# PH8411/image-matching

Measured on AMD Instinct MI355X. Metric: image-pairs/sec (640x480, 1024 kpts, 30 Sinkhorn iters), higher is better.
Workload: dtype f32

## Files before the change

### image-matching_amd/csrc/conv1ab_wino24p.hip

```cpp
#include "imx_kernels.h"
#include "wino24_h2.h"
#include <cstdint>
#include <cstdio>
#include <cstdlib>
#include <type_traits>

namespace imx {

typedef float f32x4 __attribute__((ext_vector_type(4)));
typedef float f32x2 __attribute__((ext_vector_type(2)));
typedef _Float16 f16x8 __attribute__((ext_vector_type(8)));
typedef _Float16 f16x2 __attribute__((ext_vector_type(2)));
typedef unsigned u32x4v __attribute__((ext_vector_type(4)));

namespace {
constexpr int IMG_N = IMG_H * IMG_W;

__global__ __launch_bounds__(512) void conv1ab_wino24p(ConvArgs p, int tiles_x, int tiles_y, int ntiles) {
  extern __shared__ __attribute__((aligned(16))) unsigned char smem_1p[];
  float* raw = reinterpret_cast<float*>(smem_1p + NG * VGRP * 2);
  float* img = raw + NG * RAWSZ;
  float* wmax = img + NG * IMG_N;
  unsigned* amax_tab = reinterpret_cast<unsigned*>(wmax + 8);
  const unsigned lds0 = (unsigned)(uintptr_t)(__attribute__((address_space(3))) unsigned char*)smem_1p;
// ... 271 lines not shown
    f32x4 y[2][4];
    {
      auto cols = [&](const f32x4 (&a0)[3], const f32x4 (&a1)[3], const f32x4 (&b0)[3], const f32x4 (&b1)[3]) __attribute__((always_inline)) {
        const f32x4 s0[6] = {a0[0], a0[1], a0[2], b0[0], b0[1], b0[2]}, s1[6] = {a1[0], a1[1], a1[2], b1[0], b1[1], b1[2]};
        w24_out_cols(s0, s1, k8, y);
      };
      if (ph == 0) { cols(sK0, sK1, gs0, gs1); asm volatile("" ::: "memory"); }
      else { cols(gs0, gs1, sK0, sK1); asm volatile("; order 1" ::: "memory"); }
    }
    {
      const float inv = p.u_scale_inv / sv;
      const f32x4 inv4 = {inv, inv, inv, inv};
      const f32x4 zero4 = {0.f, 0.f, 0.f, 0.f};
      const int wr = (lq & 15) >> 2, wc = lq & 3;
      const int bu = __builtin_amdgcn_readfirstlane(bcur), lv = __builtin_amdgcn_readfirstlane(lcur);
      const __amdgpu_buffer_rsrc_t ors = __builtin_amdgcn_make_buffer_rsrc((void*)(p.out + (size_t)bu * Ho * Wo * Cout), 0, lv ? Ho * Wo * Cout * 4 : 0, 0x00020000);
      const int choff = outb ? (cb * 2 + (lq >> 5)) * (Ho * Wo * 32) + ((lq >> 4) & 1) * 16 : (cb * 16 + 4 * (lq >> 4)) * 4;
      typedef unsigned u32x4 __attribute__((__vector_size__(4 * sizeof(unsigned))));
      const int oy = (y0 >> 1) + wr;
#pragma unroll
      for (int hh = 0; hh < 2; ++hh) {
        const f32x4 mx4 = __builtin_elementwise_max(__builtin_elementwise_max(y[0][2 * hh], y[0][2 * hh + 1]), __builtin_elementwise_max(y[1][2 * hh], y[1][2 * hh + 1]));
        const f32x4 v = __builtin_elementwise_max(__builtin_elementwise_fma(mx4, inv4, bs4), zero4);
        const int ox = (x0 >> 1) + 2 * wc + hh;
        const unsigned off = (oy < Ho && ox < Wo) ? (unsigned)((oy * Wo + ox) * opx + choff) : 0x7ffffff0u;
        __builtin_amdgcn_raw_buffer_store_b128(__builtin_bit_cast(u32x4, v), ors, (int)off, 0, 0);
        amax_run = max(amax_run, __builtin_bit_cast(unsigned, fmaxf(fmaxf(v[0], v[1]), fmaxf(v[2], v[3]))));
      }
      if (p.amax_out) {
        unsigned mb = amax_run;
        mb = max(mb, (unsigned)__builtin_amdgcn_update_dpp(0, (int)mb, 0xb1, 0xf, 0xf, true));
        mb = max(mb, (unsigned)__builtin_amdgcn_update_dpp(0, (int)mb, 0x4e, 0xf, 0xf, true));
        mb = max(mb, (unsigned)__builtin_amdgcn_update_dpp(0, (int)mb, 0x141, 0xf, 0xf, true));
        mb = max(mb, (unsigned)__builtin_amdgcn_update_dpp(0, (int)mb, 0x140, 0xf, 0xf, true));
        const unsigned m01 = max((unsigned)__builtin_amdgcn_readlane((int)mb, 0), (unsigned)__builtin_amdgcn_readlane((int)mb, 16));
        const unsigned m23 = max((unsigned)__builtin_amdgcn_readlane((int)mb, 32), (unsigned)__builtin_amdgcn_readlane((int)mb, 48));
        const unsigned mw = max(m01, m23);
        if (lv && mw && lq == 0) atomicMax(amax_tab + (bu & (AMAX_SLOTS - 1)), mw);
        amax_run = 0;
      }
// ... 38 lines not shown
```

### image-matching_amd/csrc/conv3x3_wino24p.hip

```cpp
#include "imx_kernels.h"
#include "wino24_h2.h"
#include <cstdint>
#include <cstdio>
#include <cstdlib>
#include <type_traits>

namespace imx {

typedef float f32x4 __attribute__((ext_vector_type(4)));
typedef float f32x2 __attribute__((ext_vector_type(2)));
typedef _Float16 f16x8 __attribute__((ext_vector_type(8)));
typedef _Float16 f16x2 __attribute__((ext_vector_type(2)));
typedef unsigned u32x4 __attribute__((ext_vector_type(4)));

namespace {
#ifdef P_TRACE
__device__ long long p_trace_buf[16 * 16];
#define P_STAMP(i_) { const long long t_ = __builtin_amdgcn_s_memtime(); tr[i_] += t_ - tlast; tlast = t_; }
#else
#define P_STAMP(i_)
#endif

struct Tile { int b, y0, x0, live; };
__device__ __forceinline__ float v_scale_inv(unsigned amax_bits) {
  unsigned e = (amax_bits >> 23) & 0xffu;
  e = e < 60u ? 60u : e > 200u ? 200u : e;
  return __builtin_bit_cast(float, (e - 8u) << 23);
}

template <bool POOL, bool RELU, bool FASTW, bool INZ>
__global__ __launch_bounds__(512) void conv3x3_wino24p(ConvArgs p, int tiles_x, int tiles_y, int ntiles, int nitems) {
  extern __shared__ __attribute__((aligned(16))) unsigned char smem_p[];
  float* raw = reinterpret_cast<float*>(smem_p + NG * VGRP * 2);
  unsigned* amax_tab = reinterpret_cast<unsigned*>(raw + NG * NSUB * RAWC);
  const unsigned lds0 = (unsigned)(uintptr_t)(__attribute__((address_space(3))) unsigned char*)smem_p;

  const int tid = threadIdx.x, lane = tid & 63;
  const int wave_s = __builtin_amdgcn_readfirstlane(tid >> 6);
  const int cb = wave_s & 3, ph = wave_s >> 2;
  const int tq = wave_s & 3, tg = wave_s >> 2;
  const int H = p.H, W = p.W, Cin = p.Cin, Cout = p.Cout;
  const int nchunk = Cin / CKH, ncob = Cout / NT;
  const int grid = (int)gridDim.x;
  const int vb = (grid & 7) == 0 ? ((int)blockIdx.x & 7) * (grid >> 3) + ((int)blockIdx.x >> 3) : (int)blockIdx.x;
  if (vb >= nitems) return;
// ... 17 lines not shown
    unsigned a = lds0 + (unsigned)(ph * (VGRP * 2) + ph * NLP * 1024 + lane * 16);
    unsigned b = lds0 + (unsigned)((1 - ph) * (VGRP * 2) + ph * NLP * 1024 + lane * 16);
    asm volatile("" : "+v"(a), "+v"(b));
    vrdK = (const _Float16*)((__attribute__((address_space(3))) unsigned char*)(uintptr_t)a);
    vrdS = (const _Float16*)((__attribute__((address_space(3))) unsigned char*)(uintptr_t)b);
  }

  auto loader_slot = [&](int t, int k, int& py, int& px_, int& half) __attribute__((always_inline)) {
    const int e = (k == 1 && t + 256 < RH * RW * 2) ? t + 256 : t;
    const int px = p.in_blocked ? e >> 1 : e % (RH * RW);
    half = p.in_blocked ? e & 1 : e / (RH * RW);
    py = px / RW - 1;
    px_ = px % RW - 1;
    return px * RSC + half * 4;
  };
  constexpr bool inz = INZ;
  auto halo_slot = [&](int t, int j, int& py, int& px_, int& piece) __attribute__((always_inline)) -> bool {
    const int hh = t + 256 * j, hp = hh >> 3;
    piece = hh & 7;
    py = hp < 18 ? 0 : hp < 36 ? RH - 1 : hp < 44 ? hp - 35 : hp - 43;
    px_ = hp < 18 ? hp : hp < 36 ? hp - 18 : hp < 44 ? 0 : RW - 1;
    return hh < 52 * 8;
  };
  int ldst[2], ldmain = 0;
  if constexpr (inz) {
    const int t = tid & 255, n = t & 15, kq = (t >> 4) & 3, x = t >> 6;
    ldmain = tg * NSUB * RAWC + (kq >> 1) * RAWC + ((1 + 2 * (n >> 2)) * RW + 1 + 4 * (n & 3) + x) * RSC + (kq & 1) * 4;
#pragma unroll
    for (int j = 0; j < 2; ++j) {
      int py, px, piece;
      halo_slot(t, j, py, px, piece);
      ldst[j] = tg * NSUB * RAWC + ((piece >> 2) * 2 + ((piece & 3) >> 1)) * RAWC + (py * RW + px) * RSC + (piece & 1) * 4;
    }
  } else {
#pragma unroll
    for (int k = 0; k < 2; ++k) { int a, b, c; ldst[k] = tg * NSUB * RAWC + loader_slot(tid & 255, k, a, b, c); }
  }
  const int cob = __builtin_amdgcn_readfirstlane(vb % ncob);
  const int dt = NG * (grid / ncob), dtx = __builtin_amdgcn_readfirstlane(dt % tiles_x), dty = __builtin_amdgcn_readfirstlane((dt / tiles_x) % tiles_y),
            dtb = __builtin_amdgcn_readfirstlane(dt / (tiles_x * tiles_y));
  Tile cur, nxt;
  {
// ... 19 lines not shown
  const int nblk_in = Cin / 16;
  const int zimg = tiles_x * tiles_y * nblk_in * 8192;
  const bool inb = p.in_blocked != 0;
  const int pxb = inb ? 8 * 4 : Cin * 4;
  const int sub_step = inb ? H * W * 8 * 4 : 8 * 4;
  auto loader_tile = [&](const Tile& t) __attribute__((always_inline)) {
    const int t8 = (wave_s & 3) * 64 + lane_now();
    int lpy[2], lpx[2], lhalf[2];
#pragma unroll
    for (int k = 0; k < 2; ++k) loader_slot(t8, k, lpy[k], lpx[k], lhalf[k]);
    const bool lv = t.live != 0;
    const int b = __builtin_amdgcn_readfirstlane(lv ? t.b : 0);
    lsv = v_scale(amax_c[b & (AMAX_SLOTS - 1)]);
    if constexpr (inz) {
      lrs = __builtin_amdgcn_make_buffer_rsrc((void*)(p.in + (size_t)b * (zimg >> 2)), 0, lv ? zimg : 0, 0x00020000);
      const int n = t8 & 15, x = t8 >> 6;
      gmain = (unsigned)((t.y0 * tiles_x + t.x0) * nblk_in * 8192 + t8 * 16);
      const bool xin = t.x0 * OW + 4 * (n & 3) + x < W;
      const int gy0 = t.y0 * OH + 2 * (n >> 2);
      mmask = ((xin && gy0 < H) ? 5u : 0u) | ((xin && gy0 + 1 < H) ? 10u : 0u);
#pragma unroll
      for (int j = 0; j < 2; ++j) {
        int py, px, piece;
        const bool used = halo_slot(t8, j, py, px, piece);
        const int gy = t.y0 * OH - 1 + py, gx = t.x0 * OW - 1 + px;
        const bool in = (int)used & (int)lv & (int)((unsigned)gy < (unsigned)H) & (int)((unsigned)gx < (unsigned)W);
        goff[j] = in ? (unsigned)((((gy >> 3) * tiles_x + (gx >> 4)) * nblk_in + (piece >> 2)) * 8192 + ((gy & 1) * 4 + (gx & 3)) * 1024 + (piece & 3) * 256 +
                                  (((gy & 7) >> 1) * 4 + ((gx & 15) >> 2)) * 16)
                     : OOB;
      }
      return;
    }
    lrs = __builtin_amdgcn_make_buffer_rsrc((void*)(p.in + (size_t)b * H * W * Cin), 0, lv ? img_bytes : 0, 0x00020000);
#pragma unroll
    for (int k = 0; k < 2; ++k) {
      const int gy = t.y0 * OH + lpy[k], gx = t.x0 * OW + lpx[k];
      const bool in = (int)lv & (int)((unsigned)gy < (unsigned)H) & (int)((unsigned)gx < (unsigned)W);
      goff[k] = in ? (unsigned)((gy * W + gx) * pxb + lhalf[k] * 16) : OOB;
    }
  };
  f32x4 rr[NSUB][2];
  float rr_sv = 1.f;
  unsigned rr_mask = 0xfu;
  auto issue_load = [&]() __attribute__((always_inline)) {
// ... 17 lines not shown
  };
  auto advance_loader = [&]() __attribute__((always_inline)) {
    if (__builtin_expect(++lchunk == nchunk, 0)) {
      lchunk = 0;
      nxt = step_tile(cur);
      if (item_c + grid >= nitems) nxt.live = 0;
      loader_tile(nxt);
      asm volatile("" ::: "memory");
    }
  };
  auto store_raw = [&]() __attribute__((always_inline)) {
    const f32x4 s4 = {rr_sv, rr_sv, rr_sv, rr_sv};
    if constexpr (inz) {
#pragma unroll
      for (int k = 0; k < 4; ++k) {
        const float mk = (rr_mask >> k) & 1u ? 1.f : 0.f;
        const f32x4 v = rr[k][0] * s4 * (f32x4){mk, mk, mk, mk};
        float* d = raw + ldmain + (k & 1) * (RW * RSC) + (k >> 1) * (2 * RAWC);
        *reinterpret_cast<f32x2*>(d) = (f32x2){v[0], v[1]};
        *reinterpret_cast<f32x2*>(d + 2) = (f32x2){v[2], v[3]};
      }
      const int t8 = (wave_s & 3) * 64 + lane_now();
#pragma unroll
      for (int j = 0; j < 2; ++j)
        if (t8 + 256 * j < 52 * 8) {
          const f32x4 v = rr[j][1] * s4;
          float* d = raw + ldst[j];
          *reinterpret_cast<f32x2*>(d) = (f32x2){v[0], v[1]};
          *reinterpret_cast<f32x2*>(d + 2) = (f32x2){v[2], v[3]};
        }
      return;
    }
#pragma unroll
// ... 182 lines not shown
      };
      if (ph == 0) { cols(sK0, sK1, gs0, gs1); asm volatile("" ::: "memory"); }
      else { cols(gs0, gs1, sK0, sK1); asm volatile("; order 1" ::: "memory"); }
    }
    P_STAMP(7)
    {
      const int lwr = (lq & 15) >> 2, lwc = lq & 3;
      const int chl = outb ? (cb * 2 + (lq >> 5)) * (Ho_k * Wo_k * 8 * 4) + ((lq >> 4) & 1) * 16 : (cb * 16 + 4 * (lq >> 4)) * 4;
      const f32x4 inv4 = {inv, inv, inv, inv};
      const f32x4 zero4 = {0.f, 0.f, 0.f, 0.f};
      const int Ho = Ho_k, Wo = Wo_k;
      typedef unsigned su32x4 __attribute__((__vector_size__(4 * sizeof(unsigned))));
      const int ibase = __builtin_amdgcn_readfirstlane(((POOL ? tl.y0 >> 1 : tl.y0) * Wo + (POOL ? tl.x0 >> 1 : tl.x0)) * opx +
                                                       (outb ? cob * (NT / 8) * (Ho * Wo * 8 * 4) : cob * NT * 4));
      const int fbase = fastw ? ibase : 0;
      const bool outz = !POOL && p.out_blocked == 2;
      const int zbase = outz ? __builtin_amdgcn_readfirstlane((((tl.y0 / OH) * tiles_x + tl.x0 / OW) * (Cout / 16) + cob * 4 + cb) * 8192) : 0;
      const size_t zimg_out = (size_t)tiles_x * tiles_y * (Cout / 16) * 2048;
      const __amdgpu_buffer_rsrc_t ors =
          outz ? __builtin_amdgcn_make_buffer_rsrc((void*)(p.out + (size_t)tl.b * zimg_out + (zbase >> 2)), 0, tl.live ? 8192 : 0, 0x00020000)
               : __builtin_amdgcn_make_buffer_rsrc((void*)(p.out + (size_t)tl.b * Ho * Wo * Cout + (fbase >> 2)), 0, tl.live ? Ho * Wo * Cout * 4 - fbase : 0, 0x00020000);
      auto note = [&](const f32x4& v) __attribute__((always_inline)) {
        const float mm = RELU ? fmaxf(fmaxf(v[0], v[1]), fmaxf(v[2], v[3])) : fmaxf(fmaxf(fabsf(v[0]), fabsf(v[1])), fmaxf(fabsf(v[2]), fabsf(v[3])));
        amax_run = max(amax_run, __builtin_bit_cast(unsigned, mm));
      };
      if constexpr (POOL) {
        const int oy = (tl.y0 >> 1) + lwr;
#pragma unroll
        for (int hh = 0; hh < 2; ++hh) {
          const f32x4 mx4 = __builtin_elementwise_max(__builtin_elementwise_max(y[0][2 * hh], y[0][2 * hh + 1]), __builtin_elementwise_max(y[1][2 * hh], y[1][2 * hh + 1]));
          f32x4 v = __builtin_elementwise_fma(mx4, inv4, bs4);
          if (RELU) v = __builtin_elementwise_max(v, zero4);
          note(v);
          const int ox = (tl.x0 >> 1) + 2 * lwc + hh;
          const int so_ = (lwr * Wo + 2 * lwc + hh) * opx + chl;
          const unsigned off = fastw ? (unsigned)so_ : (oy < Ho && ox < Wo) ? (unsigned)(so_ + ibase) : OOB;
          __builtin_amdgcn_raw_buffer_store_b128(__builtin_bit_cast(su32x4, v), ors, (int)off, 0, 0);
        }
      } else {
#pragma unroll
        for (int r = 0; r < 2; ++r)
#pragma unroll
          for (int x = 0; x < 4; ++x) {
            f32x4 v = __builtin_elementwise_fma(y[r][x], inv4, bs4);
            if (RELU) v = __builtin_elementwise_max(v, zero4);
            note(v);
            const int oy = tl.y0 + 2 * lwr + r, ox = tl.x0 + 4 * lwc + x;
            const int so_ = ((2 * lwr + r) * Wo + 4 * lwc + x) * opx + chl;
            const unsigned off = outz ? (unsigned)((r * 4 + x) * 1024 + lq * 16) : fastw ? (unsigned)so_ : (oy < Ho && ox < Wo) ? (unsigned)(so_ + ibase) : OOB;
            __builtin_amdgcn_raw_buffer_store_b128(__builtin_bit_cast(su32x4, v), ors, (int)off, 0, 0);
          }
      }
      P_STAMP(13)
      if (p.amax_out) {
        unsigned mb = amax_run;
        mb = max(mb, (unsigned)__builtin_amdgcn_update_dpp(0, (int)mb, 0xb1, 0xf, 0xf, true));
        mb = max(mb, (unsigned)__builtin_amdgcn_update_dpp(0, (int)mb, 0x4e, 0xf, 0xf, true));
        mb = max(mb, (unsigned)__builtin_amdgcn_update_dpp(0, (int)mb, 0x141, 0xf, 0xf, true));
        mb = max(mb, (unsigned)__builtin_amdgcn_update_dpp(0, (int)mb, 0x140, 0xf, 0xf, true));
        const unsigned m01 = max((unsigned)__builtin_amdgcn_readlane((int)mb, 0), (unsigned)__builtin_amdgcn_readlane((int)mb, 16));
        const unsigned m23 = max((unsigned)__builtin_amdgcn_readlane((int)mb, 32), (unsigned)__builtin_amdgcn_readlane((int)mb, 48));
        const unsigned mw = max(m01, m23);
        if (tl.live && mw && lq == 0) atomicMax(amax_tab + (tl.b & (AMAX_SLOTS - 1)), mw);
        amax_run = 0;
// ... 8 lines not shown
    __syncthreads();
    for (int i = tid; i < AMAX_SLOTS; i += 512)
      if (amax_tab[i]) atomicMax(p.amax_out + i, amax_tab[i]);
  }
#ifdef P_TRACE
#ifdef P_TRACE_WAVES
  if (lane == 0 && blockIdx.x == 0)
    for (int i = 0; i < 16; ++i) p_trace_buf[wave_s * 16 + i] = tr[i];
#else
  if (tid == 0 && (blockIdx.x & 15) == 0 && (blockIdx.x >> 4) < 16)
    for (int i = 0; i < 16; ++i) p_trace_buf[(blockIdx.x >> 4) * 16 + i] = tr[i];
#endif
#endif
}

template <bool POOL, bool RELU, bool FASTW, bool INZ>
hipError_t launch_p2(const ConvArgs& a, hipStream_t s) {
  const int tiles_x = (a.W + OW - 1) / OW, tiles_y = (a.H + OH - 1) / OH;
  const int ntiles = tiles_x * tiles_y * a.B;
  const int nitems = ((ntiles + NG - 1) / NG) * (a.Cout / NT);
  const size_t lds = (size_t)NG * VGRP * 2 + (size_t)NG * NSUB * RAWC * sizeof(float) + AMAX_SLOTS * sizeof(unsigned);
  const int ncu = device_cu_count();
  if (!ncu) return hipErrorUnknown;
  auto k = conv3x3_wino24p<POOL, RELU, FASTW, INZ>;
  static unsigned long long attr = 0;
  raise_lds_limit(reinterpret_cast<const void*>(k), (int)lds, attr);
  const int ncob = a.Cout / NT;
  const dim3 grid((unsigned)(nitems <= ncu ? nitems : ncu - ncu % ncob));
  if (grid.x == 0) return hipErrorInvalidValue;
  last_form = "conv3x3_wino24p:f16x2";
  hipLaunchKernelGGL(k, grid, dim3(512), lds, s, a, tiles_x, tiles_y, ntiles, nitems);
  return hipGetLastError();
}
template <bool POOL, bool RELU, bool FASTW>
hipError_t launch_p(const ConvArgs& a, hipStream_t s) {
  return a.in_blocked == 2 ? launch_p2<POOL, RELU, FASTW, true>(a, s) : launch_p2<POOL, RELU, FASTW, false>(a, s);
}
}

#ifdef P_TRACE
void conv_p_trace_read(long long* out) { (void)hipMemcpyFromSymbol(out, HIP_SYMBOL(p_trace_buf), sizeof(long long) * 16 * 16); }
#endif

bool conv3x3_wino24p_supported(const ConvArgs& a) {
  if (!conv3x3_wino24h_supported(a)) return false;
  const size_t padded = (size_t)((a.H + OH - 1) / OH * OH) * ((a.W + OW - 1) / OW * OW) * 4;
  return padded * a.Cin < (size_t)OOB && padded * a.Cout < (size_t)OOB;
}

bool conv3x3_wino24p_preferred(const ConvArgs& a) {
  if (!conv3x3_wino24p_supported(a)) return false;
// ... 19 lines not shown
```

### image-matching_amd/csrc/imx_api.cpp

```cpp
#include "imx_host.h"

#include <dlfcn.h>

#include <atomic>
#include <memory>

namespace imx {
thread_local const char* last_form = nullptr;
}

namespace {
bool ends_with(const std::string& s, const std::string& suf) {
  return s.size() >= suf.size() && s.compare(s.size() - suf.size(), suf.size(), suf) == 0;
}
}

extern "C" {

#ifndef IMX_BUILD_ID
#define IMX_BUILD_ID "dev"
#endif
const char* imx_version(void) { return "imx 0.4 gfx950 hip-7.2 fp32 build " IMX_BUILD_ID; }

int imx_create(int device_id, const imx_config_t* cfg, imx_handle_t* out) {
// ... 409 lines not shown
    if (shape_out) for (size_t i = 0; i < it->second.shape.size() && i < 4; ++i) shape_out[i] = it->second.shape[i];
    if (!host_out) return 0;
    if (capacity < n) return fail(h, "imx_debug_fetch: capacity %lld < %lld elements", (long long)capacity, (long long)n);
    HIP_OK(h, hipSetDevice(h->device));
    HIP_OK(h, hipDeviceSynchronize());
    if (h->nms_lazy.pending && name && std::string(name) == "nms") {
      auto& z = h->nms_lazy;
      HIP_OK(h, launch_nms(z.smap, z.nms, z.B, z.H, z.W, z.radius, nullptr, z.scratch));
      HIP_OK(h, hipDeviceSynchronize());
      z.pending = false;
    }
    if (!it->second.blocked) {
      HIP_OK(h, hipMemcpy(host_out, it->second.p, (size_t)n * 4, hipMemcpyDeviceToHost));
      return 0;
    }
    std::vector<float> raw((size_t)n);
    HIP_OK(h, hipMemcpy(raw.data(), it->second.p, (size_t)n * 4, hipMemcpyDeviceToHost));
    const int64_t Bn = it->second.shape[0], Hn = it->second.shape[1], Wn = it->second.shape[2], Cn = it->second.shape[3];
    for (int64_t bb = 0; bb < Bn; ++bb)
      for (int64_t ck = 0; ck < Cn / 8; ++ck)
        for (int64_t yx = 0; yx < Hn * Wn; ++yx)
          for (int64_t c = 0; c < 8; ++c)
            host_out[(bb * Hn * Wn + yx) * Cn + ck * 8 + c] = raw[((bb * (Cn / 8) + ck) * Hn * Wn + yx) * 8 + c];
    return 0;
  });
}

int imx_set_timing(imx_handle_t h, int enable) {
  return guarded(h, "imx_set_timing", [&]() -> int {
    if (!h) return -1;
    h->timing = enable != 0;
    return 0;
  });
}

int imx_timing_reset(imx_handle_t h) {
  return guarded(h, "imx_timing_reset", [&]() -> int {
    if (!h) return -1;
// ... 62 lines not shown
```

### image-matching_amd/csrc/imx_host.h

```cpp
#pragma once
#include "../../include/imx.h"
#include "imx_kernels.h"
#include "gnn_tail_pack.h"

#include <hip/hip_runtime.h>

#include <algorithm>
#include <cstdarg>
#include <cstdio>
#include <exception>
#include <map>
#include <new>
#include <string>
#include <vector>

namespace imx::host {

constexpr int HEADS = 4;

struct HostTensor {
  std::vector<float> data;
  std::vector<int64_t> shape;
};
struct DevBuf {
// ... 19 lines not shown
  float* b = nullptr;
  int K = 0, N = 0, Npad = 0;
};
struct GnnLayer {
  GemmW qkv, merge, mlp1, mlp2;
  float* tail_stream = nullptr;
  void* tail_stream_h2 = nullptr;
  GnnTailH2Consts h2c{};
  float bmax_1 = 0.f, bmax_2 = 0.f;
  float qkv_spread = 1.f;
};
struct Tap {
  const void* p;
  std::vector<int64_t> shape;
  bool blocked = false;
};
struct TimedEvent {
  std::string name;
  const char* form;
  hipEvent_t e0, e1;
};
struct TimingRow {
  std::string name, form;
  int64_t launches;
  double ms;
};

inline std::string g_create_error;

}
// ... 211 lines not shown
```

### image-matching_amd/csrc/imx_superpoint.cpp

```cpp
#include "imx_host.h"

namespace imx::host {

namespace {

struct SpLayer { const char* name; int level; bool pool, first, last, swz; };
constexpr int kSpN = 8;
constexpr SpLayer kSpLayers[kSpN] = {{"conv1ab_pool", 0, true, true, false, false}, {"conv2a", 1, false, false, false, true},
                                  {"conv2b_pool", 1, true, false, false, false}, {"conv3a", 2, false, false, false, true},
                                  {"conv3b_pool", 2, true, false, false, false}, {"conv4a", 3, false, false, false, true},
                                  {"conv4b", 3, false, false, false, false},     {"convPaDa", 3, false, false, true, false}};
constexpr int kSlice = 256;

struct SpWork {
  int B, H, W, split;
  const float *img0, *img1;
  float* act[kSpN];
  unsigned* amax;
};
enum class ConvForm : unsigned char { Direct, Wino, WinoH, WinoP, C1, C1H, C1P };
constexpr hipError_t (*kConvLaunch[])(const ConvArgs&, hipStream_t) = {launch_conv3x3, launch_conv3x3_wino24, launch_conv3x3_wino24h, launch_conv3x3_wino24p,
                                                                       launch_conv1ab_wino24, launch_conv1ab_wino24h, launch_conv1ab_wino24p};
static_assert(sizeof(kConvLaunch) / sizeof(*kConvLaunch) == (size_t)ConvForm::C1P + 1, "one launcher per ConvForm, in the enum's order");
struct SpStep { ConvForm form; unsigned char in_blocked, out_blocked; };
struct SpPlan {
  bool blocked;
  bool chain;
  int nslice;
  int heads_cout;
  SpStep steps[2][kSpN];
};

ConvArgs conv_args(imx_handle_t h, const SpWork& w, const SpPlan& P, int li, int sl) {
  const SpLayer& T = kSpLayers[li];
  const ConvW& cw = h->conv[li];
  const int hh = w.H >> T.level, ww = w.W >> T.level, cout = T.last ? P.heads_cout : cw.cout;
  const int b0 = P.chain ? sl * kSlice : 0, nb = P.chain ? std::min(kSlice, w.B - b0) : w.B;
  const size_t ztile = (size_t)((hh + 7) / 8) * ((ww + 15) / 16) * 2048;
  const size_t in_img = li && kSpLayers[li - 1].swz ? ztile * (cw.cin / 16) : (size_t)hh * ww * (T.first ? 1 : cw.cin);
  const size_t out_img = T.swz ? ztile * (cout / 16) : (size_t)(T.pool ? hh / 2 : hh) * (T.pool ? ww / 2 : ww) * cout;
  ConvArgs a{};
  if (P.chain) {
    unsigned* am = w.amax + (size_t)sl * kSpN * 256;
    a.amax_out = T.last ? nullptr : am + (size_t)li * 256;
    a.amax_in = li > 0 ? am + (size_t)(li - 1) * 256 : nullptr;
    a.wuh = cw.wuh; a.u_scale_inv = cw.su_inv;
    a.c1a_l1 = h->c1a_l1; a.c1a_bmax = h->c1a_bmax;
  }
  a.in = (li ? w.act[li - 1] : w.img0) + (size_t)b0 * in_img;
  if (T.first) {
    if (b0 >= w.split) { a.in = w.img1 + (size_t)(b0 - w.split) * in_img; a.split = nb; }
    else { a.in2 = w.img1; a.split = w.split - b0; }
  }
  a.w = cw.w; a.wu24 = cw.wu24; a.bias = cw.b; a.w1 = h->w1; a.b1 = h->b1; a.out = w.act[li] + (size_t)b0 * out_img;
  a.B = nb; a.H = hh; a.W = ww; a.Cin = cw.cin; a.Cout = cout; a.relu = 1; a.pool = T.pool; a.first = T.first;
// ... 19 lines not shown
    const ConvArgs a = conv_args(h, w, P, kSpN - 1, 0);
    if (!conv3x3_wino24_supported(a) || (P.chain && !conv3x3_wino24h_supported(a))) P.heads_cout = h->conv[kSpN - 1].cout;
  }
  if (P.chain) P.nslice = (w.B + kSlice - 1) / kSlice;
  const bool pairs = P.chain && o.conv_f16 == 1;
  for (int r = P.nslice > 1 ? 0 : 1; r < 2; ++r) {
    SpStep* st = P.steps[r];
    for (int li = 0; li < kSpN; ++li) {
      st[li] = SpStep{};
      const ConvArgs a = conv_args(h, w, P, li, r ? P.nslice - 1 : 0);
      if (li ? !wino[li] : o.conv_direct) st[li].form = ConvForm::Direct;
      else if (li) st[li].form = !P.chain ? ConvForm::Wino : pairs && conv3x3_wino24p_preferred(a) ? ConvForm::WinoP : ConvForm::WinoH;
      else st[li].form = !(P.chain && conv1ab_wino24h_supported(a)) ? ConvForm::C1 : pairs && conv1ab_wino24p_preferred(a) ? ConvForm::C1P : ConvForm::C1H;
    }
    for (int li = 0; li < kSpN; ++li) {
      const bool swz = kSpLayers[li].swz && o.conv_swizzle != 0 && st[li].form == ConvForm::WinoP && st[li + 1].form == ConvForm::WinoP;
      st[li].out_blocked = swz ? 2 : (P.blocked && !kSpLayers[li].last) ? 1 : 0;
      if (li + 1 < kSpN) st[li + 1].in_blocked = st[li].out_blocked;
    }
  }
}

}

int sp_detect(imx_handle_t h, const float* img0, const float* img1, int split, int B, int H, int W, int32_t* counts_out,
              hipStream_t s, bool dense_only, int32_t* counts_lo, int32_t* counts_hi, bool det_only) {
  if (!h->finalized[IMX_NET_SUPERPOINT]) return fail(h, "SuperPoint weights not finalized");
  h->nms_lazy.pending = false;
  if (B <= 0 || H < 8 || W < 8) return fail(h, "bad image batch shape B=%d H=%d W=%d", B, H, W);
  const imx_config_t& c = h->cfg;
  const int H2 = H / 2, W2 = W / 2, H4 = H2 / 2, W4 = W2 / 2, Hc = H4 / 2, Wc = W4 / 2, H8 = Hc * 8, W8 = Wc * 8;
  const int d = c.descriptor_dim;
  const size_t f = sizeof(float);
  WS(a1, float, "sp.a1", (size_t)B * H2 * W2 * 64 * f);
  auto padded = [](int hh, int ww) { return (size_t)((hh + 7) / 8 * 8) * ((ww + 15) / 16 * 16); };
  WS(a2a, float, "sp.a2a", (size_t)B * padded(H2, W2) * 64 * f);
  WS(a2, float, "sp.a2", (size_t)B * H4 * W4 * 64 * f);
  WS(a3a, float, "sp.a3a", (size_t)B * padded(H4, W4) * 128 * f);
  WS(a3, float, "sp.a3", (size_t)B * Hc * Wc * 128 * f);
  WS(a4a, float, "sp.a4a", (size_t)B * padded(Hc, Wc) * 128 * f);
  WS(x4, float, "sp.x4", (size_t)B * Hc * Wc * 128 * f);
  WS(hd, float, "sp.heads", (size_t)B * Hc * Wc * 512 * f);
  WS(semi, float, "sp.semi", (size_t)B * Hc * Wc * 65 * f);
  float* dense = nullptr;
  if (!det_only) {
    WS(dense_, float, "sp.dense", (size_t)B * Hc * Wc * d * f);
    dense = dense_;
  }
  const bool kp_bits = nms_candidate_bits_supported(c.nms_radius, c.keypoint_threshold) && h->opt.keypoints != 0;
  SpWork w{B, H, W, split, img0, img1, {a1, a2a, a2, a3a, a3, a4a, x4, hd}, nullptr};
  const size_t amax_bytes = (size_t)((B + kSlice - 1) / kSlice) * kSpN * 256 * 4;
  if (!h->opt.conv_direct && conv_chain_h_ok(h) && h->opt.conv_f16 && !h->opt.mfma_f32) {
    WS(am, unsigned, "sp.amax", amax_bytes);
    w.amax = am;
  }
  SpPlan P;
// ... 34 lines not shown
  WS(sel_count, int, "kp.sel_count", (size_t)B * 4);
  WS(sel_idx, int, "kp.sel_idx", (size_t)B * Ksel * 4);
  WS(sel_score, float, "kp.sel_score", (size_t)B * Ksel * 4);
  k.row_count = row_count; k.row_off = row_off; k.cand_count = cand_count; k.cand_idx = cand_idx; k.cand_score = cand_score;
  k.sel_count = sel_count; k.sel_idx = sel_idx; k.sel_score = sel_score;
  k.counts_out[0] = counts_out; k.counts_out[1] = counts_lo; k.counts_out[2] = counts_hi; k.counts_split = split;
  if (c.max_keypoints > 16384) {
    size_t P = 1;
    while (P < (size_t)c.max_keypoints) P <<= 1;
    WS(slots, unsigned long long, "kp.sort_slots", (size_t)B * P * 8);
    k.sort_scratch = slots;
  }
  RUN("keypoints", launch_keypoints(k, s));

  h->det_B = B; h->det_H = H; h->det_W = W; h->det_Hc = Hc; h->det_Wc = Wc; h->det_Ksel = Ksel;
  tap(h, "a1", a1, {B, H2, W2, 64}, blocked);
  tap(h, "a2", a2, {B, H4, W4, 64}, blocked);
  tap(h, "a3", a3, {B, Hc, Wc, 128}, blocked);
  tap(h, "x4", x4, {B, Hc, Wc, 128}, blocked);
  tap(h, "semi", semi, {B, Hc, Wc, 65});
  tap(h, "desc_raw", dense, {B, Hc, Wc, d});
  tap(h, "score_map", smap, {B, H8, W8});
  h->nms_lazy.smap = smap; h->nms_lazy.nms = nms; h->nms_lazy.scratch = nms_scratch; h->nms_lazy.B = B; h->nms_lazy.H = H8; h->nms_lazy.W = W8;
  h->nms_lazy.radius = c.nms_radius; h->nms_lazy.pending = kp_bits;
  tap(h, "nms", nms, {B, H8, W8});
  return 0;
}

int sp_describe(imx_handle_t h, int b0, int B, int Kcap, float* kpts, float* scores, float* desc, hipStream_t s,
                int split, float* kpts2, float* scores2, float* desc2) {
  if (h->det_B <= 0 || b0 + B > h->det_B) return fail(h, "describe: no matching imx_superpoint_detect (B=%d, detect B=%d)", B, h->det_B);
  DescribeArgs a{};
  a.dense = static_cast<const float*>(h->bufs["sp.dense"].p);
  a.ld = h->cfg.descriptor_dim; a.d = h->cfg.descriptor_dim; a.Hc = h->det_Hc; a.Wc = h->det_Wc; a.W8 = h->det_Wc * 8;
// ... 12 lines not shown
```

Measured before the change: 2579.

## Extend tile-swizzled activation layout to pooled producers and conv4b output

Adds a new tile-swizzled layout (3) for pooling conv producers, including conv1ab, so that each pooled output tile is written as a contiguous quadrant of the consumer's 8x16 tile block. The consumer Winograd loader is templated on the layout so it can read the new form directly, and conv4b now also emits the existing swizzled layout. The aim is to replace scattered NHWC-style stores and halo gathers with contiguous block transfers across more layers of the chain. Activation buffers are padded to whole tiles, and the host tap de-swizzle is generalised to handle mixed layouts across slices.

Result: no change. 2572 (-0.3%).

```diff
diff --git a/image-matching_amd/csrc/conv1ab_wino24p.hip b/image-matching_amd/csrc/conv1ab_wino24p.hip
--- a/image-matching_amd/csrc/conv1ab_wino24p.hip
+++ b/image-matching_amd/csrc/conv1ab_wino24p.hip
@@ -1,5 +1,6 @@
 #include "imx_kernels.h"
 #include "wino24_h2.h"
+#include "tile_swizzle.h"
 #include <cstdint>
 #include <cstdio>
 #include <cstdlib>
@@ -309,7 +310,13 @@
       const f32x4 zero4 = {0.f, 0.f, 0.f, 0.f};
       const int wr = (lq & 15) >> 2, wc = lq & 3;
       const int bu = __builtin_amdgcn_readfirstlane(bcur), lv = __builtin_amdgcn_readfirstlane(lcur);
-      const __amdgpu_buffer_rsrc_t ors = __builtin_amdgcn_make_buffer_rsrc((void*)(p.out + (size_t)bu * Ho * Wo * Cout), 0, lv ? Ho * Wo * Cout * 4 : 0, 0x00020000);
+      const bool outz = p.out_blocked == 3;
+      const int pty = __builtin_amdgcn_readfirstlane(y0) / OH, ptx = __builtin_amdgcn_readfirstlane(x0) / OW, ztiles_x = (Wo + OW - 1) / OW, ztiles_y = (Ho + OH - 1) / OH;
+      const bool zlive = lv && (pty >> 1) < ztiles_y && (ptx >> 1) < ztiles_x;
+      const int zbase = outz ? __builtin_amdgcn_readfirstlane(zswz_block(pty >> 1, ptx >> 1, ztiles_x, Cout / 16, cb) + zswz_quadrant(pty, ptx)) : 0;
+      const __amdgpu_buffer_rsrc_t ors =
+          outz ? __builtin_amdgcn_make_buffer_rsrc((void*)(p.out + (size_t)bu * zswz_image_floats(Ho, Wo, Cout) + (zbase >> 2)), 0, zlive ? kZQuadBytes : 0, 0x00020000)
+               : __builtin_amdgcn_make_buffer_rsrc((void*)(p.out + (size_t)bu * Ho * Wo * Cout), 0, lv ? Ho * Wo * Cout * 4 : 0, 0x00020000);
       const int choff = outb ? (cb * 2 + (lq >> 5)) * (Ho * Wo * 32) + ((lq >> 4) & 1) * 16 : (cb * 16 + 4 * (lq >> 4)) * 4;
       typedef unsigned u32x4 __attribute__((__vector_size__(4 * sizeof(unsigned))));
       const int oy = (y0 >> 1) + wr;
@@ -318,7 +325,7 @@
         const f32x4 mx4 = __builtin_elementwise_max(__builtin_elementwise_max(y[0][2 * hh], y[0][2 * hh + 1]), __builtin_elementwise_max(y[1][2 * hh], y[1][2 * hh + 1]));
         const f32x4 v = __builtin_elementwise_max(__builtin_elementwise_fma(mx4, inv4, bs4), zero4);
         const int ox = (x0 >> 1) + 2 * wc + hh;
-        const unsigned off = (oy < Ho && ox < Wo) ? (unsigned)((oy * Wo + ox) * opx + choff) : 0x7ffffff0u;
+        const unsigned off = outz ? (unsigned)(zswz_store3(hh) + lq * 16) : (oy < Ho && ox < Wo) ? (unsigned)((oy * Wo + ox) * opx + choff) : 0x7ffffff0u;
         __builtin_amdgcn_raw_buffer_store_b128(__builtin_bit_cast(u32x4, v), ors, (int)off, 0, 0);
         amax_run = max(amax_run, __builtin_bit_cast(unsigned, fmaxf(fmaxf(v[0], v[1]), fmaxf(v[2], v[3]))));
       }
diff --git a/image-matching_amd/csrc/conv3x3_wino24p.hip b/image-matching_amd/csrc/conv3x3_wino24p.hip
--- a/image-matching_amd/csrc/conv3x3_wino24p.hip
+++ b/image-matching_amd/csrc/conv3x3_wino24p.hip
@@ -1,5 +1,6 @@
 #include "imx_kernels.h"
 #include "wino24_h2.h"
+#include "tile_swizzle.h"
 #include <cstdint>
 #include <cstdio>
 #include <cstdlib>
@@ -28,7 +29,7 @@
   return __builtin_bit_cast(float, (e - 8u) << 23);
 }
 
-template <bool POOL, bool RELU, bool FASTW, bool INZ>
+template <bool POOL, bool RELU, bool FASTW, int INL>
 __global__ __launch_bounds__(512) void conv3x3_wino24p(ConvArgs p, int tiles_x, int tiles_y, int ntiles, int nitems) {
   extern __shared__ __attribute__((aligned(16))) unsigned char smem_p[];
   float* raw = reinterpret_cast<float*>(smem_p + NG * VGRP * 2);
@@ -76,7 +77,7 @@
     px_ = px % RW - 1;
     return px * RSC + half * 4;
   };
-  constexpr bool inz = INZ;
+  constexpr bool inz = INL != 0;
   auto halo_slot = [&](int t, int j, int& py, int& px_, int& piece) __attribute__((always_inline)) -> bool {
     const int hh = t + 256 * j, hp = hh >> 3;
     piece = hh & 7;
@@ -86,8 +87,9 @@
   };
   int ldst[2], ldmain = 0;
   if constexpr (inz) {
-    const int t = tid & 255, n = t & 15, kq = (t >> 4) & 3, x = t >> 6;
-    ldmain = tg * NSUB * RAWC + (kq >> 1) * RAWC + ((1 + 2 * (n >> 2)) * RW + 1 + 4 * (n & 3) + x) * RSC + (kq & 1) * 4;
+    const int t = tid & 255;
+    const ZPixel q = zswz_unpixel<INL>(t);
+    ldmain = tg * NSUB * RAWC + (q.kq >> 1) * RAWC + ((1 + q.y) * RW + 1 + q.x) * RSC + (q.kq & 1) * 4;
 #pragma unroll
     for (int j = 0; j < 2; ++j) {
       int py, px, piece;
@@ -137,20 +139,18 @@
     lsv = v_scale(amax_c[b & (AMAX_SLOTS - 1)]);
     if constexpr (inz) {
       lrs = __builtin_amdgcn_make_buffer_rsrc((void*)(p.in + (size_t)b * (zimg >> 2)), 0, lv ? zimg : 0, 0x00020000);
-      const int n = t8 & 15, x = t8 >> 6;
-      gmain = (unsigned)((t.y0 * tiles_x + t.x0) * nblk_in * 8192 + t8 * 16);
-      const bool xin = t.x0 * OW + 4 * (n & 3) + x < W;
-      const int gy0 = t.y0 * OH + 2 * (n >> 2);
-      mmask = ((xin && gy0 < H) ? 5u : 0u) | ((xin && gy0 + 1 < H) ? 10u : 0u);
+      const ZPixel q = zswz_unpixel<INL>(t8);
+      gmain = (unsigned)(zswz_block(t.y0, t.x0, tiles_x, nblk_in, 0) + t8 * 16);
+      const bool xin = t.x0 * OW + q.x < W;
+      const int gy0 = t.y0 * OH + q.y;
+      mmask = ((xin && gy0 < H) ? 5u : 0u) | ((xin && gy0 + kZRowStep<INL> < H) ? 10u : 0u);
 #pragma unroll
       for (int j = 0; j < 2; ++j) {
         int py, px, piece;
         const bool used = halo_slot(t8, j, py, px, piece);
         const int gy = t.y0 * OH - 1 + py, gx = t.x0 * OW - 1 + px;
         const bool in = (int)used & (int)lv & (int)((unsigned)gy < (unsigned)H) & (int)((unsigned)gx < (unsigned)W);
-        goff[j] = in ? (unsigned)((((gy >> 3) * tiles_x + (gx >> 4)) * nblk_in + (piece >> 2)) * 8192 + ((gy & 1) * 4 + (gx & 3)) * 1024 + (piece & 3) * 256 +
-                                  (((gy & 7) >> 1) * 4 + ((gx & 15) >> 2)) * 16)
-                     : OOB;
+        goff[j] = in ? (unsigned)(zswz_block(gy >> 3, gx >> 4, tiles_x, nblk_in, piece >> 2) + zswz_pixel<INL>(gy & 7, gx & 15, piece & 3)) : OOB;
       }
       return;
     }
@@ -198,9 +198,12 @@
     if constexpr (inz) {
 #pragma unroll
       for (int k = 0; k < 4; ++k) {
-        const float mk = (rr_mask >> k) & 1u ? 1.f : 0.f;
-        const f32x4 v = rr[k][0] * s4 * (f32x4){mk, mk, mk, mk};
-        float* d = raw + ldmain + (k & 1) * (RW * RSC) + (k >> 1) * (2 * RAWC);
+        const bool in = (rr_mask >> k) & 1u;
+        const float mk = in ? 1.f : 0.f;
+        f32x4 v = rr[k][0] * s4;
+        if constexpr (INL == 3) v = in ? v : (f32x4){0.f, 0.f, 0.f, 0.f};
+        else v = v * (f32x4){mk, mk, mk, mk};
+        float* d = raw + ldmain + (k & 1) * (kZRowStep<INL> * RW * RSC) + (k >> 1) * (2 * RAWC);
         *reinterpret_cast<f32x2*>(d) = (f32x2){v[0], v[1]};
         *reinterpret_cast<f32x2*>(d + 2) = (f32x2){v[2], v[3]};
       }
@@ -413,11 +416,14 @@
       const int ibase = __builtin_amdgcn_readfirstlane(((POOL ? tl.y0 >> 1 : tl.y0) * Wo + (POOL ? tl.x0 >> 1 : tl.x0)) * opx +
                                                        (outb ? cob * (NT / 8) * (Ho * Wo * 8 * 4) : cob * NT * 4));
       const int fbase = fastw ? ibase : 0;
-      const bool outz = !POOL && p.out_blocked == 2;
-      const int zbase = outz ? __builtin_amdgcn_readfirstlane((((tl.y0 / OH) * tiles_x + tl.x0 / OW) * (Cout / 16) + cob * 4 + cb) * 8192) : 0;
-      const size_t zimg_out = (size_t)tiles_x * tiles_y * (Cout / 16) * 2048;
+      const bool outz = p.out_blocked == (POOL ? 3 : 2);
+      const int pty = tl.y0 / OH, ptx = tl.x0 / OW, zty = POOL ? pty >> 1 : pty, ztx = POOL ? ptx >> 1 : ptx;
+      const int ztiles_x = (Wo_k + OW - 1) / OW, ztiles_y = (Ho_k + OH - 1) / OH;
+      const bool zlive = tl.live && zty < ztiles_y && ztx < ztiles_x;
+      const int zbase = outz ? __builtin_amdgcn_readfirstlane(zswz_block(zty, ztx, ztiles_x, Cout / 16, cob * 4 + cb) + (POOL ? zswz_quadrant(pty, ptx) : 0)) : 0;
+      const size_t zimg_out = zswz_image_floats(Ho_k, Wo_k, Cout);
       const __amdgpu_buffer_rsrc_t ors =
-          outz ? __builtin_amdgcn_make_buffer_rsrc((void*)(p.out + (size_t)tl.b * zimg_out + (zbase >> 2)), 0, tl.live ? 8192 : 0, 0x00020000)
+          outz ? __builtin_amdgcn_make_buffer_rsrc((void*)(p.out + (size_t)tl.b * zimg_out + (zbase >> 2)), 0, zlive ? (POOL ? kZQuadBytes : kZBlockBytes) : 0, 0x00020000)
                : __builtin_amdgcn_make_buffer_rsrc((void*)(p.out + (size_t)tl.b * Ho * Wo * Cout + (fbase >> 2)), 0, tl.live ? Ho * Wo * Cout * 4 - fbase : 0, 0x00020000);
       auto note = [&](const f32x4& v) __attribute__((always_inline)) {
         const float mm = RELU ? fmaxf(fmaxf(v[0], v[1]), fmaxf(v[2], v[3])) : fmaxf(fmaxf(fabsf(v[0]), fabsf(v[1])), fmaxf(fabsf(v[2]), fabsf(v[3])));
@@ -433,7 +439,7 @@
           note(v);
           const int ox = (tl.x0 >> 1) + 2 * lwc + hh;
           const int so_ = (lwr * Wo + 2 * lwc + hh) * opx + chl;
-          const unsigned off = fastw ? (unsigned)so_ : (oy < Ho && ox < Wo) ? (unsigned)(so_ + ibase) : OOB;
+          const unsigned off = outz ? (unsigned)(zswz_store3(hh) + lq * 16) : fastw ? (unsigned)so_ : (oy < Ho && ox < Wo) ? (unsigned)(so_ + ibase) : OOB;
           __builtin_amdgcn_raw_buffer_store_b128(__builtin_bit_cast(su32x4, v), ors, (int)off, 0, 0);
         }
       } else {
@@ -446,7 +452,7 @@
             note(v);
             const int oy = tl.y0 + 2 * lwr + r, ox = tl.x0 + 4 * lwc + x;
             const int so_ = ((2 * lwr + r) * Wo + 4 * lwc + x) * opx + chl;
-            const unsigned off = outz ? (unsigned)((r * 4 + x) * 1024 + lq * 16) : fastw ? (unsigned)so_ : (oy < Ho && ox < Wo) ? (unsigned)(so_ + ibase) : OOB;
+            const unsigned off = outz ? (unsigned)(zswz_store2(r, x) + lq * 16) : fastw ? (unsigned)so_ : (oy < Ho && ox < Wo) ? (unsigned)(so_ + ibase) : OOB;
             __builtin_amdgcn_raw_buffer_store_b128(__builtin_bit_cast(su32x4, v), ors, (int)off, 0, 0);
           }
       }
@@ -485,7 +491,7 @@
 #endif
 }
 
-template <bool POOL, bool RELU, bool FASTW, bool INZ>
+template <bool POOL, bool RELU, bool FASTW, int INL>
 hipError_t launch_p2(const ConvArgs& a, hipStream_t s) {
   const int tiles_x = (a.W + OW - 1) / OW, tiles_y = (a.H + OH - 1) / OH;
   const int ntiles = tiles_x * tiles_y * a.B;
@@ -493,7 +499,7 @@
   const size_t lds = (size_t)NG * VGRP * 2 + (size_t)NG * NSUB * RAWC * sizeof(float) + AMAX_SLOTS * sizeof(unsigned);
   const int ncu = device_cu_count();
   if (!ncu) return hipErrorUnknown;
-  auto k = conv3x3_wino24p<POOL, RELU, FASTW, INZ>;
+  auto k = conv3x3_wino24p<POOL, RELU, FASTW, INL>;
   static unsigned long long attr = 0;
   raise_lds_limit(reinterpret_cast<const void*>(k), (int)lds, attr);
   const int ncob = a.Cout / NT;
@@ -505,7 +511,8 @@
 }
 template <bool POOL, bool RELU, bool FASTW>
 hipError_t launch_p(const ConvArgs& a, hipStream_t s) {
-  return a.in_blocked == 2 ? launch_p2<POOL, RELU, FASTW, true>(a, s) : launch_p2<POOL, RELU, FASTW, false>(a, s);
+  if (a.in_blocked == 3) return launch_p2<POOL, RELU, FASTW, 3>(a, s);
+  return a.in_blocked == 2 ? launch_p2<POOL, RELU, FASTW, 2>(a, s) : launch_p2<POOL, RELU, FASTW, 0>(a, s);
 }
 }
 
diff --git a/image-matching_amd/csrc/imx_api.cpp b/image-matching_amd/csrc/imx_api.cpp
--- a/image-matching_amd/csrc/imx_api.cpp
+++ b/image-matching_amd/csrc/imx_api.cpp
@@ -447,14 +447,28 @@
       HIP_OK(h, hipMemcpy(host_out, it->second.p, (size_t)n * 4, hipMemcpyDeviceToHost));
       return 0;
     }
-    std::vector<float> raw((size_t)n);
-    HIP_OK(h, hipMemcpy(raw.data(), it->second.p, (size_t)n * 4, hipMemcpyDeviceToHost));
-    const int64_t Bn = it->second.shape[0], Hn = it->second.shape[1], Wn = it->second.shape[2], Cn = it->second.shape[3];
-    for (int64_t bb = 0; bb < Bn; ++bb)
-      for (int64_t ck = 0; ck < Cn / 8; ++ck)
-        for (int64_t yx = 0; yx < Hn * Wn; ++yx)
-          for (int64_t c = 0; c < 8; ++c)
-            host_out[(bb * Hn * Wn + yx) * Cn + ck * 8 + c] = raw[((bb * (Cn / 8) + ck) * Hn * Wn + yx) * 8 + c];
+    const Tap& t = it->second;
+    const int64_t Bn = t.shape[0], Hn = t.shape[1], Wn = t.shape[2], Cn = t.shape[3];
+    const int64_t zimg = (int64_t)zswz_image_floats((int)Hn, (int)Wn, (int)Cn), bimg = Hn * Wn * Cn;
+    const int64_t slice = t.slice > 0 ? t.slice : Bn, region = t.slice > 0 ? zimg : bimg;
+    std::vector<float> raw((size_t)(Bn * region));
+    HIP_OK(h, hipMemcpy(raw.data(), t.p, raw.size() * 4, hipMemcpyDeviceToHost));
+    const int tiles_x = (int)(Wn + 15) / 16, nblk = (int)Cn / 16;
+    for (int64_t bb = 0; bb < Bn; ++bb) {
+      const int64_t sl = bb / slice;
+      const int L = t.layout[(sl + 1) * slice >= Bn];
+      const float* img = raw.data() + sl * slice * region + (bb - sl * slice) * (L >= 2 ? zimg : bimg);
+      float* out = host_out + bb * bimg;
+      for (int64_t y = 0; y < Hn; ++y)
+        for (int64_t x = 0; x < Wn; ++x)
+          for (int64_t c = 0; c < Cn; ++c) {
+            const int blk = (int)c / 16, kq = (int)(c >> 2) & 3;
+            const int64_t src = L == 2   ? (zswz_block((int)y >> 3, (int)x >> 4, tiles_x, nblk, blk) + zswz_pixel<2>((int)y & 7, (int)x & 15, kq)) / 4 + (c & 3)
+                                : L == 3 ? (zswz_block((int)y >> 3, (int)x >> 4, tiles_x, nblk, blk) + zswz_pixel<3>((int)y & 7, (int)x & 15, kq)) / 4 + (c & 3)
+                                         : ((c / 8) * Hn * Wn + y * Wn + x) * 8 + (c & 7);
+            out[(y * Wn + x) * Cn + c] = img[src];
+          }
+    }
     return 0;
   });
 }
diff --git a/image-matching_amd/csrc/imx_host.h b/image-matching_amd/csrc/imx_host.h
--- a/image-matching_amd/csrc/imx_host.h
+++ b/image-matching_amd/csrc/imx_host.h
@@ -1,6 +1,7 @@
 #pragma once
 #include "../../include/imx.h"
 #include "imx_kernels.h"
+#include "tile_swizzle.h"
 #include "gnn_tail_pack.h"
 
 #include <hip/hip_runtime.h>
@@ -57,6 +58,7 @@
   const void* p;
   std::vector<int64_t> shape;
   bool blocked = false;
+  int layout[2] = {1, 1}, slice = 0;
 };
 struct TimedEvent {
   std::string name;
diff --git a/image-matching_amd/csrc/imx_superpoint.cpp b/image-matching_amd/csrc/imx_superpoint.cpp
--- a/image-matching_amd/csrc/imx_superpoint.cpp
+++ b/image-matching_amd/csrc/imx_superpoint.cpp
@@ -4,12 +4,12 @@
 
 namespace {
 
-struct SpLayer { const char* name; int level; bool pool, first, last, swz; };
+struct SpLayer { const char* name; int level; bool pool, first, last; int swz; };
 constexpr int kSpN = 8;
-constexpr SpLayer kSpLayers[kSpN] = {{"conv1ab_pool", 0, true, true, false, false}, {"conv2a", 1, false, false, false, true},
-                                  {"conv2b_pool", 1, true, false, false, false}, {"conv3a", 2, false, false, false, true},
-                                  {"conv3b_pool", 2, true, false, false, false}, {"conv4a", 3, false, false, false, true},
-                                  {"conv4b", 3, false, false, false, false},     {"convPaDa", 3, false, false, true, false}};
+constexpr SpLayer kSpLayers[kSpN] = {{"conv1ab_pool", 0, true, true, false, 3}, {"conv2a", 1, false, false, false, 2},
+                                  {"conv2b_pool", 1, true, false, false, 3}, {"conv3a", 2, false, false, false, 2},
+                                  {"conv3b_pool", 2, true, false, false, 3}, {"conv4a", 3, false, false, false, 2},
+                                  {"conv4b", 3, false, false, false, 2},     {"convPaDa", 3, false, false, true, 0}};
 constexpr int kSlice = 256;
 
 struct SpWork {
@@ -36,9 +36,9 @@
   const ConvW& cw = h->conv[li];
   const int hh = w.H >> T.level, ww = w.W >> T.level, cout = T.last ? P.heads_cout : cw.cout;
   const int b0 = P.chain ? sl * kSlice : 0, nb = P.chain ? std::min(kSlice, w.B - b0) : w.B;
-  const size_t ztile = (size_t)((hh + 7) / 8) * ((ww + 15) / 16) * 2048;
-  const size_t in_img = li && kSpLayers[li - 1].swz ? ztile * (cw.cin / 16) : (size_t)hh * ww * (T.first ? 1 : cw.cin);
-  const size_t out_img = T.swz ? ztile * (cout / 16) : (size_t)(T.pool ? hh / 2 : hh) * (T.pool ? ww / 2 : ww) * cout;
+  const int ho = T.pool ? hh / 2 : hh, wo = T.pool ? ww / 2 : ww;
+  const size_t in_img = li && kSpLayers[li - 1].swz ? zswz_image_floats(hh, ww, cw.cin) : (size_t)hh * ww * (T.first ? 1 : cw.cin);
+  const size_t out_img = T.swz ? zswz_image_floats(ho, wo, cout) : (size_t)ho * wo * cout;
   ConvArgs a{};
   if (P.chain) {
     unsigned* am = w.amax + (size_t)sl * kSpN * 256;
@@ -88,8 +88,8 @@
       else st[li].form = !(P.chain && conv1ab_wino24h_supported(a)) ? ConvForm::C1 : pairs && conv1ab_wino24p_preferred(a) ? ConvForm::C1P : ConvForm::C1H;
     }
     for (int li = 0; li < kSpN; ++li) {
-      const bool swz = kSpLayers[li].swz && o.conv_swizzle != 0 && st[li].form == ConvForm::WinoP && st[li + 1].form == ConvForm::WinoP;
-      st[li].out_blocked = swz ? 2 : (P.blocked && !kSpLayers[li].last) ? 1 : 0;
+      const bool swz = kSpLayers[li].swz && o.conv_swizzle != 0 && (st[li].form == ConvForm::WinoP || st[li].form == ConvForm::C1P) && st[li + 1].form == ConvForm::WinoP;
+      st[li].out_blocked = swz ? kSpLayers[li].swz : (P.blocked && !kSpLayers[li].last) ? 1 : 0;
       if (li + 1 < kSpN) st[li + 1].in_blocked = st[li].out_blocked;
     }
   }
@@ -106,14 +106,14 @@
   const int H2 = H / 2, W2 = W / 2, H4 = H2 / 2, W4 = W2 / 2, Hc = H4 / 2, Wc = W4 / 2, H8 = Hc * 8, W8 = Wc * 8;
   const int d = c.descriptor_dim;
   const size_t f = sizeof(float);
-  WS(a1, float, "sp.a1", (size_t)B * H2 * W2 * 64 * f);
   auto padded = [](int hh, int ww) { return (size_t)((hh + 7) / 8 * 8) * ((ww + 15) / 16 * 16); };
+  WS(a1, float, "sp.a1", (size_t)B * padded(H2, W2) * 64 * f);
   WS(a2a, float, "sp.a2a", (size_t)B * padded(H2, W2) * 64 * f);
-  WS(a2, float, "sp.a2", (size_t)B * H4 * W4 * 64 * f);
+  WS(a2, float, "sp.a2", (size_t)B * padded(H4, W4) * 64 * f);
   WS(a3a, float, "sp.a3a", (size_t)B * padded(H4, W4) * 128 * f);
-  WS(a3, float, "sp.a3", (size_t)B * Hc * Wc * 128 * f);
+  WS(a3, float, "sp.a3", (size_t)B * padded(Hc, Wc) * 128 * f);
   WS(a4a, float, "sp.a4a", (size_t)B * padded(Hc, Wc) * 128 * f);
-  WS(x4, float, "sp.x4", (size_t)B * Hc * Wc * 128 * f);
+  WS(x4, float, "sp.x4", (size_t)B * padded(Hc, Wc) * 128 * f);
   WS(hd, float, "sp.heads", (size_t)B * Hc * Wc * 512 * f);
   WS(semi, float, "sp.semi", (size_t)B * Hc * Wc * 65 * f);
   float* dense = nullptr;
@@ -178,10 +178,18 @@
   RUN("keypoints", launch_keypoints(k, s));
 
   h->det_B = B; h->det_H = H; h->det_W = W; h->det_Hc = Hc; h->det_Wc = Wc; h->det_Ksel = Ksel;
-  tap(h, "a1", a1, {B, H2, W2, 64}, blocked);
-  tap(h, "a2", a2, {B, H4, W4, 64}, blocked);
-  tap(h, "a3", a3, {B, Hc, Wc, 128}, blocked);
-  tap(h, "x4", x4, {B, Hc, Wc, 128}, blocked);
+  auto act_tap = [&](const char* name, int li, const float* p, std::vector<int64_t> shape) {
+    tap(h, name, p, std::move(shape), blocked);
+    if (blocked) {
+      Tap& t = h->taps[name];
+      t.layout[0] = P.steps[P.nslice > 1 ? 0 : 1][li].out_blocked; t.layout[1] = P.steps[1][li].out_blocked;
+      t.slice = P.chain ? kSlice : 0;
+    }
+  };
+  act_tap("a1", 0, a1, {B, H2, W2, 64});
+  act_tap("a2", 2, a2, {B, H4, W4, 64});
+  act_tap("a3", 4, a3, {B, Hc, Wc, 128});
+  act_tap("x4", 6, x4, {B, Hc, Wc, 128});
   tap(h, "semi", semi, {B, Hc, Wc, 65});
   tap(h, "desc_raw", dense, {B, Hc, Wc, d});
   tap(h, "score_map", smap, {B, H8, W8});
diff --git a/image-matching_amd/csrc/tile_swizzle.h b/image-matching_amd/csrc/tile_swizzle.h
--- /dev/null
+++ b/image-matching_amd/csrc/tile_swizzle.h
@@ -0,0 +1,60 @@
+#pragma once
+#include <cstddef>
+
+namespace imx {
+
+constexpr int kZBlockBytes = 8192;
+constexpr int kZQuadBytes = 2048;
+
+constexpr size_t zswz_image_floats(int H, int W, int C) { return (size_t)((H + 7) / 8) * ((W + 15) / 16) * (C / 16) * (kZBlockBytes / 4); }
+constexpr int zswz_block(int tile_y, int tile_x, int tiles_x, int nblk, int blk) { return ((tile_y * tiles_x + tile_x) * nblk + blk) * kZBlockBytes; }
+
+template <int L>
+constexpr int zswz_pixel(int y, int x, int kq) {
+  static_assert(L == 2 || L == 3, "tile-swizzled layouts: 2 (no pool), 3 (pooled producer)");
+  return L == 2 ? ((y & 1) * 4 + (x & 3)) * 1024 + kq * 256 + ((y >> 1) * 4 + (x >> 2)) * 16
+                : ((y >> 2) * 2 + (x >> 3)) * 2048 + (x & 1) * 1024 + kq * 256 + ((y & 3) * 4 + ((x & 7) >> 1)) * 16;
+}
+struct ZPixel { int y, x, kq; };
+template <int L>
+constexpr ZPixel zswz_unpixel(int e) {
+  const int n = e & 15, kq = (e >> 4) & 3, s = e >> 6;
+  return L == 2 ? ZPixel{2 * (n >> 2) + (s >> 2), 4 * (n & 3) + (s & 3), kq} : ZPixel{4 * (s >> 2) + (n >> 2), 8 * ((s >> 1) & 1) + 2 * (n & 3) + (s & 1), kq};
+}
+template <int L>
+constexpr int kZRowStep = L == 2 ? 1 : 4;
+
+constexpr int zswz_store2(int r, int x) { return (r * 4 + x) * 1024; }
+constexpr int zswz_store3(int hh) { return hh * 1024; }
+constexpr int zswz_quadrant(int prod_tile_y, int prod_tile_x) { return ((prod_tile_y & 1) * 2 + (prod_tile_x & 1)) * kZQuadBytes; }
+
+namespace zswz_check {
+constexpr bool stores_agree() {
+  for (int lane = 0; lane < 64; ++lane) {
+    const int n = lane & 15, kq = lane >> 4, wr = n >> 2, wc = n & 3;
+    for (int r = 0; r < 2; ++r)
+      for (int x = 0; x < 4; ++x)
+        if (zswz_store2(r, x) + lane * 16 != zswz_pixel<2>(2 * wr + r, 4 * wc + x, kq)) return false;
+    for (int ty = 0; ty < 2; ++ty)
+      for (int tx = 0; tx < 2; ++tx)
+        for (int hh = 0; hh < 2; ++hh)
+          if (zswz_quadrant(ty, tx) + zswz_store3(hh) + lane * 16 != zswz_pixel<3>(4 * ty + wr, 8 * tx + 2 * wc + hh, kq)) return false;
+  }
+  return true;
+}
+template <int L>
+constexpr bool inverse_agrees() {
+  for (int e = 0; e < 512; ++e) {
+    const ZPixel q = zswz_unpixel<L>(e);
+    if (zswz_pixel<L>(q.y, q.x, q.kq) != e * 16) return false;
+    if (e < 256) {
+      const ZPixel d = zswz_unpixel<L>(e + 256);
+      if (d.y != q.y + kZRowStep<L> || d.x != q.x || d.kq != q.kq) return false;
+    }
+  }
+  return true;
+}
+static_assert(stores_agree() && inverse_agrees<2>() && inverse_agrees<3>(), "tile_swizzle.h: stores, loader and de-swizzle disagree");
+}
+
+}
```
